# yamrom/smash-paper

Measured on AMD Instinct MI355X. Metric: reads/sec mapped+binned (hg19, 150 bp) at 1/2/4/8 MI355X; bit-exact bin counts, higher is better.
Workload: dtype u8/u64 (integer); 1 GPU; C3 hg19-shaped, 50 M x 150 bp SMASH reads per rank (25 M pairs, one run in batches), sample_bins/50000; genome=hg19, index_words=packed (SA / ISA hints, DESIGN section 3), genome_bp=3095693983, text_N=6191388016, pairs_per_rank=25000000, read_len=150, batch_pairs=12500000, bins=50000, parallelism=single GPU

## Files before the change

### smash-paper_amd/csrc/mam_sm.hpp

```cpp
#pragma once
#include "mam_device.hpp"

#ifndef PAD_KEEP
#define PAD_KEEP(x) asm volatile("" : "+v"(x))
#endif
#ifndef SM_KNOB
#define SM_KNOB(field, dflt) (dflt)
#endif
#ifndef SM_HOOK_BM
#define SM_HOOK_BM(mode, a1, a2)
#endif
#ifndef SM_HOOK_F
#define SM_HOOK_F(j, bits)
#endif
#ifndef SM_HOOK_BS
#define SM_HOOK_BS(size, depth)
#endif
#ifndef SM_HOOK_CMPBS
#define SM_HOOK_CMPBS(begin, sp, off)
#endif
#ifndef SM_HOOK_RUN
#define SM_HOOK_RUN(begin, kind, ext_l, ext_r)
#endif
#ifndef SM_HOOK_BYTE
#define SM_HOOK_BYTE(pos)
#endif
#ifndef SM_HOOK_PARK
#define SM_HOOK_PARK(a)
#endif
#ifndef SM_LOAD16
#define SM_LOAD16(a) ::smash::sm::load16u(a)
#endif
#ifndef SM_LOAD16ST
#define SM_LOAD16ST(a, st) SM_LOAD16(a)
#endif
#ifndef SM_LOADPF16
#define SM_LOADPF16(a) ::smash::sm::load16u(a)
#endif
#ifndef SM_LOADIDX
#define SM_LOADIDX(p, i) uint64_t((p)[i])
#endif
#ifndef SM_HOOK_PF
#define SM_HOOK_PF(a)
#endif
#ifndef SM_PERM
#define SM_PERM(s0, s1, sel) __builtin_amdgcn_perm(s0, s1, sel)
#endif

#ifndef SM_REGION
#define SM_REGION(k)                                                              \
  do {                                                                            \
    if (STATS) {                                                                  \
      const uint64_t am_ = __ballot(1);                                           \
      if (lane == uint32_t(__builtin_ctzll(am_))) atomicAdd(c.wave_stats + 64 + (k), 1ull); \
    }                                                                             \
  } while (0)
#endif

#ifndef SM_DMA_ROW
#define SM_DMA_ROW(dst, src, n, lane) ::smash::sm::dma_row(dst, src, n, lane)
#endif

namespace smash {
namespace sm {

#ifdef SM_DMA_ROW_HOST
__device__ __forceinline__ uint4 load16u(uint64_t a) {
  uint4 v;
  __builtin_memcpy(&v, reinterpret_cast<const uint8_t *>(a), 16);
  return v;
}
#else
typedef uint32_t sm_u32x4 __attribute__((ext_vector_type(4)));
typedef sm_u32x4 sm_u32x4_u __attribute__((aligned(1)));
typedef __attribute__((address_space(1))) const sm_u32x4_u glb_block16_t;
__device__ __forceinline__ uint4 load16u(uint64_t a) {
  const sm_u32x4 b = *reinterpret_cast<glb_block16_t *>(a);
  return make_uint4(b.x, b.y, b.z, b.w);
}
#endif

#ifndef SM_DMA_ROW_HOST
typedef __attribute__((address_space(3))) void lds_void_t;
typedef __attribute__((address_space(1))) const void glb_void_t;
__device__ __forceinline__ void dma_row(uint32_t *dst, const uint4 *src, uint32_t n, uint32_t lane) {
  if (lane < n)
    __builtin_amdgcn_global_load_lds((glb_void_t *)(src + lane), (lds_void_t *)dst, 16, 0, 0);
}
#endif

struct Geom {
  uint32_t w_raw;
  uint32_t w_row;
  uint32_t c_bad;
  uint32_t chunks;
};

__host__ __device__ constexpr uint32_t geo_row(uint32_t L) {
  return ((L + 11) / 4 + 3) / 4 * 4 < 8 ? 8u : ((L + 11) / 4 + 3) / 4 * 4;
}

inline Geom make_geom(uint32_t max_len) {
  Geom g;
  g.w_raw = (max_len + 11) / 4;
  g.w_row = (g.w_raw + 3) & ~3u;
  if (g.w_row < 8) g.w_row = 8;
  g.c_bad = max_len > 128 ? 2 : 1;
  g.chunks = g.c_bad + (g.w_row + 3) / 4;
  return g;
}


inline uint32_t prep_per_block(const Geom &g, uint64_t stride) {
  const uint64_t per = 24 * 1024 / (stride + 4 * (g.chunks * 4) + 8);
  return uint32_t(per < 1 ? 1 : per > 64 ? 64 : per);
}
__host__ __device__ inline uint32_t prep_in_words(uint64_t stride, uint32_t per) {
  return (uint32_t((per * stride + 8 + 3) / 4 + 10) + 3) & ~3u;
}
inline size_t prep_lds_bytes(const Geom &g, uint64_t stride, uint32_t per) {
  return size_t(prep_in_words(stride, per)) * 4 + size_t(per) * (g.chunks * 4) * 4;
}

__global__ __launch_bounds__(256) void k_prep(const uint8_t *__restrict__ seqs, uint64_t stride,
                                              const uint16_t *__restrict__ lens, uint32_t len0,
                                              uint64_t n, uint64_t it0, uint64_t it1, uint64_t it2,
                                              uint64_t it3, Geom g, uint32_t per,
                                              uint32_t *__restrict__ rec) {
  extern __shared__ uint32_t prep_lds[];
  const uint32_t rw = g.chunks * 4;
  const uint32_t G = 4 * g.c_bad;
  const uint64_t r0 = uint64_t(blockIdx.x) * per;
  if (r0 >= n) return;
  const uint32_t nr = uint32_t(n - r0 < per ? n - r0 : per);
  const uint64_t a0 = reinterpret_cast<uint64_t>(seqs + r0 * stride);
  const uint64_t a1 = reinterpret_cast<uint64_t>(seqs + (r0 + nr) * stride);
  const uint64_t w0 = a0 & ~uint64_t(3);
  const uint32_t nw = uint32_t(((a1 + 3) & ~uint64_t(3)) - w0) / 4;
  uint32_t *in = prep_lds;
  uint32_t *out = prep_lds + prep_in_words(stride, per);
  uint32_t k0 = 0;
  if ((w0 & 15) == 0) {
    const uint32_t n4 = nw / 4;
    for (uint32_t k = threadIdx.x; k < n4; k += blockDim.x)
      reinterpret_cast<uint4 *>(in)[k] = reinterpret_cast<const uint4 *>(w0)[k];
    k0 = 4 * n4;
  }
  for (uint32_t k = k0 + threadIdx.x; k < nw; k += blockDim.x)
    in[k] = reinterpret_cast<const uint32_t *>(w0)[k];
  for (uint32_t k = threadIdx.x; k < nr * rw / 4; k += blockDim.x)
    reinterpret_cast<uint4 *>(out)[k] = make_uint4(0, 0, 0, 0);
  __syncthreads();
  auto itx = [&](uint32_t b) {
    const uint64_t w = b < 64 ? it0 : b < 128 ? it1 : b < 192 ? it2 : it3;
    return uint32_t((w >> (b & 63)) & 1ull);
  };
  const uint32_t ia = itx('a'), ic = itx('c'), ig = itx('g'), iu = itx('t');
  for (uint32_t item = threadIdx.x; item < nr * G; item += blockDim.x) {
    const uint32_t t = item / G, gi = item - t * G;
    const uint32_t L = lens ? lens[r0 + t] : len0;
    if (32 * gi >= L) continue;
    const uint32_t boff = uint32_t(a0 - w0) + uint32_t(t * stride) + 32 * gi;
    const uint32_t wq = boff >> 2, sh = (boff & 3) * 8;
    uint32_t *o = out + t * rw;
    uint32_t bw = 0;
#pragma unroll
    for (uint32_t k = 0; k < 8; ++k) {
      uint32_t w = in[wq + k];
      if (sh) w = (w >> sh) | (in[wq + k + 1] << (32 - sh));
      const uint32_t i0 = 32 * gi + 4 * k;
#pragma unroll
      for (uint32_t j = 0; j < 4; ++j) {
        const uint32_t b = (w >> (8 * j)) & 0xFF;
        const bool live = i0 + j < L;
        if (!live) w &= ~(0xFFu << (8 * j));
        const uint32_t good = (b == 'a' ? ia : 0u) | (b == 'c' ? ic : 0u) |
                              (b == 'g' ? ig : 0u) | (b == 't' ? iu : 0u);
        bw |= uint32_t(live && !good) << (4 * k + j);
      }
      if (8 * gi + k < g.w_raw) o[4 * g.c_bad + 8 * gi + k] = w;
    }
    o[gi] = bw;
  }
  __syncthreads();
  uint4 *dst = reinterpret_cast<uint4 *>(rec + r0 * rw);
  for (uint32_t k = threadIdx.x; k < nr * rw / 4; k += blockDim.x)
    dst[k] = reinterpret_cast<const uint4 *>(out)[k];
}

__global__ __launch_bounds__(256) void k_prep_direct(const uint8_t *__restrict__ seqs,
                                                     uint64_t stride,
                                                     const uint16_t *__restrict__ lens,
                                                     uint32_t len0, uint32_t n, uint32_t ga,
                                                     uint64_t it0, uint64_t it1, uint64_t it2,
                                                     uint64_t it3, Geom g,
                                                     uint32_t *__restrict__ rec, uint32_t prio) {
#ifndef SM_DMA_ROW_HOST
  if (prio) __builtin_amdgcn_s_setprio(2);
#endif
  const uint32_t item = blockIdx.x * blockDim.x + threadIdx.x;
  if (item >= n * ga) return;
  const uint32_t r = item / ga;
  const uint32_t gi = item - r * ga;
  const uint32_t L = lens ? lens[r] : len0;
  uint32_t *o = rec + uint64_t(r) * (g.chunks * 4);
  uint32_t w8[8] = {0, 0, 0, 0, 0, 0, 0, 0};
  uint32_t bw = 0;
  if (32 * gi < L) {
    auto itx = [&](uint32_t b) {
      const uint64_t w = b < 64 ? it0 : b < 128 ? it1 : b < 192 ? it2 : it3;
      return uint32_t((w >> (b & 63)) & 1ull);
    };
    const uint32_t ia = itx('a'), ic = itx('c'), ig = itx('g'), iu = itx('t');
    const uint64_t end = reinterpret_cast<uint64_t>(seqs) + uint64_t(n) * stride;
    const uint64_t b0 = reinterpret_cast<uint64_t>(seqs) + uint64_t(r) * stride + 32 * gi;
    const uint64_t a16 = b0 & ~uint64_t(15);
    const uint32_t off = uint32_t(b0 & 15);
    uint32_t d[12];
#pragma unroll
    for (uint32_t k = 0; k < 3; ++k) {
      const uint4 v = a16 + 16 * k < end && (k < 2 || off) ? reinterpret_cast<const uint4 *>(a16)[k]
                                                          : make_uint4(0, 0, 0, 0);
      d[4 * k] = v.x; d[4 * k + 1] = v.y; d[4 * k + 2] = v.z; d[4 * k + 3] = v.w;
    }
    const uint32_t q = off >> 2, sh = (off & 3) * 8;
#pragma unroll
    for (uint32_t k = 0; k < 8; ++k) {
      const uint32_t lo = q == 0 ? d[k] : q == 1 ? d[k + 1] : q == 2 ? d[k + 2] : d[k + 3];
      const uint32_t hi = q == 0 ? d[k + 1] : q == 1 ? d[k + 2] : q == 2 ? d[k + 3] : d[k + 4];
      uint32_t w = sh ? (lo >> sh) | (hi << (32 - sh)) : lo;
      const uint32_t i0 = 32 * gi + 4 * k;
#pragma unroll
      for (uint32_t j = 0; j < 4; ++j) {
        const uint32_t b = (w >> (8 * j)) & 0xFF;
        const bool live = i0 + j < L;
        if (!live) w &= ~(0xFFu << (8 * j));
        const uint32_t good = (b == 'a' ? ia : 0u) | (b == 'c' ? ic : 0u) |
                              (b == 'g' ? ig : 0u) | (b == 't' ? iu : 0u);
        bw |= uint32_t(live && !good) << (4 * k + j);
      }
      w8[k] = 8 * gi + k < g.w_raw ? w : 0u;
    }
  }
  o[gi] = bw;
  uint32_t *raw = o + 4 * g.c_bad;
  if (8 * gi + 8 <= g.w_row) {
    reinterpret_cast<uint4 *>(raw + 8 * gi)[0] = make_uint4(w8[0], w8[1], w8[2], w8[3]);
    reinterpret_cast<uint4 *>(raw + 8 * gi)[1] = make_uint4(w8[4], w8[5], w8[6], w8[7]);
  } else {
#pragma unroll
    for (uint32_t k = 0; k < 8; ++k)
      if (8 * gi + k < g.w_row) raw[8 * gi + k] = w8[k];
  }
  if (gi == ga - 1) {
    for (uint32_t k = ga; k < 4 * g.c_bad; ++k) o[k] = 0;
    for (uint32_t k = 8 * ga; k < g.w_row; ++k) raw[k] = 0;
  }
}

inline uint32_t prep_groups(uint32_t max_len) { return (max_len + 31) / 32; }

enum : uint32_t { S_EXIT = 0, S_NEW, S_ALU, S_COPY, S_BM, S_KT, S_IDX, S_BYTE, S_CMP, S_USCAN,
                  S_EXL, S_EXR, S_EXB };
enum : uint32_t { O_SAPOS, O_SAPOS2, O_BS_SA, O_ISAJ, O_NS_SA2, O_NS_ISA2 };
enum : uint32_t { O_EXT = 0, O_BS };
enum : uint32_t { A_NONE = 0, A_BSP, A_BS, A_BS_DONE, A_XL_DONE, A_RUN_DONE, A_CHAIN_DONE,
                  A_EXPAND, A_AFTER, A_TOP, A_TRAV, A_DONE, A_EMIT, A_EXS,
                  A_TOPR };
enum : uint32_t { BS_INSERT = 0, BS_LEFT, BS_RIGHT };

__device__ __forceinline__ uint64_t lo64(const uint4 &v) { return uint64_t(v.x) | (uint64_t(v.y) << 32); }
__device__ __forceinline__ uint64_t hi64(const uint4 &v) { return uint64_t(v.z) | (uint64_t(v.w) << 32); }
__device__ __forceinline__ uint32_t dword_at(const uint4 &v, uint32_t i) {
  return i == 0 ? v.x : i == 1 ? v.y : i == 2 ? v.z : v.w;
}
__device__ __forceinline__ uint32_t byte_at(const uint4 &v, uint32_t o) {
  return (dword_at(v, o >> 2) >> (8 * (o & 3))) & 0xFF;
}
__device__ __forceinline__ uint64_t bytes8_at(const uint4 &v, uint32_t o) {
  const uint64_t lo = lo64(v), hi = hi64(v);
  if (o == 0) return lo;
  if (o < 8) return (lo >> (8 * o)) | (hi << (64 - 8 * o));
  if (o == 8) return hi;
  return hi >> (8 * (o - 8));
}
__device__ __forceinline__ uint32_t agree_block(const uint4 &v, uint32_t o, const uint8_t *P,
                                                uint32_t poff, uint32_t lim) {
  uint32_t k = agree8(bytes8_at(v, o), lds_load8(P, poff), lim < 8 ? lim : 8u);
  if (k == 8 && lim > 8) k += agree8(bytes8_at(v, o + 8), lds_load8(P, poff + 8), lim - 8);
  return k;
}
template <class F>
__device__ __forceinline__ uint32_t byte_mask(const uint4 &v, F f) {
  uint32_t m = 0;
#pragma unroll
  for (uint32_t i = 0; i < 16; ++i) {
    const uint32_t b = (dword_at(v, i >> 2) >> (8 * (i & 3))) & 0xFF;
    m |= uint32_t(f(b, i)) << i;
  }
  return m;
}

#ifndef SM_PK_SUB16
typedef unsigned short sm_u16x2 __attribute__((ext_vector_type(2)));
__device__ __forceinline__ uint32_t pk_sub16(uint32_t a, uint32_t b) {
  return __builtin_bit_cast(uint32_t, __builtin_bit_cast(sm_u16x2, a) - __builtin_bit_cast(sm_u16x2, b));
}
#define SM_PK_SUB16(a, b) ::smash::sm::pk_sub16(a, b)
#endif

__device__ __forceinline__ uint32_t gt4(uint32_t w, uint32_t te, uint32_t to) {
  const uint32_t e = SM_PERM(w, w, 0x0c020c00u), o = SM_PERM(w, w, 0x0c030c01u);
  const uint32_t r = SM_PERM(SM_PK_SUB16(to, o), SM_PK_SUB16(te, e), 0x0b090a08u);
  return ((r & 0x80808080u) * 0x00204081u) >> 28;
}
__device__ __forceinline__ uint32_t thr_mask(const uint4 &v, uint32_t base, bool desc) {
  const uint32_t bp = base * 0x00010001u, s4 = desc ? 0x00040004u : 0u;
  uint32_t te = bp - (desc ? 0x00020000u : 0u), to = bp - (desc ? 0x00030001u : 0u);
  uint32_t m = 0;
#pragma unroll
  for (uint32_t k = 0; k < 4; ++k) {
    m |= gt4(dword_at(v, k), te, to) << (4 * k);
    te -= s4;
    to -= s4;
  }
  return m;
}

struct FlagRef {
  uint32_t &f;
  uint32_t b;
  __device__ __forceinline__ operator bool() const { return (f >> b) & 1u; }
  __device__ __forceinline__ FlagRef &operator=(bool x) {
    f = (f & ~(1u << b)) | (uint32_t(x) << b);
    return *this;
  }
  __device__ __forceinline__ FlagRef &operator=(const FlagRef &o) { return *this = bool(o); }
};

struct Bad {
  uint32_t w0, w1, w2, w3, w4, w5, w6, w7;
  __device__ __forceinline__ uint32_t word(uint32_t i) const {
    uint32_t r = 0;
    r = i == 0 ? w0 : r; r = i == 1 ? w1 : r; r = i == 2 ? w2 : r; r = i == 3 ? w3 : r;
    r = i == 4 ? w4 : r; r = i == 5 ? w5 : r; r = i == 6 ? w6 : r; r = i == 7 ? w7 : r;
    return r;
  }
  __device__ __forceinline__ uint32_t bits(uint32_t a, uint32_t n) const {
    const uint32_t q = a >> 5, s = a & 31;
    const uint64_t x = (uint64_t(word(q + 1)) << 32) | word(q);
    const uint32_t y = uint32_t(x >> s);
    return n >= 32 ? y : (y & ((1u << n) - 1));
  }
  __device__ __forceinline__ uint64_t bits64(uint32_t a) const {
    const uint32_t q = a >> 5, s = a & 31;
    const uint64_t x = (uint64_t(word(q + 1)) << 32) | word(q);
    const uint64_t z = uint64_t(word(q + 2)) << 32;
    return (x >> s) | (s ? z << (32 - s) : 0ull);
  }
  __device__ __forceinline__ int32_t last(uint32_t a, uint32_t n) const {
    uint32_t e = a + n;
    while (e > a) {
      const uint32_t k = e - a < 32 ? e - a : 32u;
      const uint32_t s = e - k;
      const uint32_t y = bits(s, k);
      if (y) return int32_t(s + 31 - __builtin_clz(y));
      e = s;
    }
    return -1;
  }
};

__device__ __forceinline__ uint32_t byte4_codes(uint32_t w) {
  const uint32_t cb = SM_PERM(0x02000003u, 0x01000000u, w & 0x07070707u);
  return (cb * 0x40100401u) >> 24;
}

__device__ __forceinline__ uint64_t codes_raw(const uint32_t *R, uint32_t w_row, uint32_t p,
                                              uint32_t n) {
  const uint32_t q0 = p >> 2, qm = w_row - 6;
  const uint32_t q = q0 < qm ? q0 : qm, sh = p - 4 * q;
  uint32_t hi = byte4_codes(R[q]);
  hi = (hi << 8) | byte4_codes(R[q + 1]);
  hi = (hi << 8) | byte4_codes(R[q + 2]);
  hi = (hi << 8) | byte4_codes(R[q + 3]);
  const uint32_t lo = (byte4_codes(R[q + 4]) << 8) | byte4_codes(R[q + 5]);
  const uint64_t x = (uint64_t(hi) << 16) | lo;
  return (x >> (48 - 2 * (sh + n))) & ((1ull << (2 * n)) - 1);
}

__device__ __forceinline__ uint64_t codes_raw7(const uint32_t *R, uint32_t w_row, uint32_t p,
                                               uint32_t n) {
  const uint32_t q0 = p >> 2, qm = w_row - 7;
  const uint32_t q = q0 < qm ? q0 : qm, sh = p - 4 * q;
  uint32_t hi = byte4_codes(R[q]);
  hi = (hi << 8) | byte4_codes(R[q + 1]);
  hi = (hi << 8) | byte4_codes(R[q + 2]);
  uint32_t lo = byte4_codes(R[q + 3]);
  lo = (lo << 8) | byte4_codes(R[q + 4]);
  lo = (lo << 8) | byte4_codes(R[q + 5]);
  lo = (lo << 8) | byte4_codes(R[q + 6]);
  const uint64_t x = (uint64_t(hi) << 32) | lo;
  return (x >> (56 - 2 * (sh + n))) & ((1ull << (2 * n)) - 1);
}

template <class IdxT>
struct Ctx {
  const uint8_t *T;
  const IdxT *SA, *ISA;
  const uint8_t *L8, *U;
  const uint64_t *KT;
  uint64_t N;
  uint32_t logN, K, B, min_len;
  const uint4 *rec;
  uint32_t chunks, c_bad, w_row, w_raw;
  const uint4 *rows;
  uint32_t direct;
  uint32_t bad_tab_lo, bad_tab_hi;
  uint32_t lin_blocks;
  uint32_t pad;
  uint32_t mhint;
  uint32_t grab;
  uint32_t bm_dual;
  uint32_t pf;
  uint32_t u32;
  uint32_t f2;
  const uint16_t *lens;
  uint32_t len0, cap;
  uint64_t n_reads;
  uint64_t *out;
  uint32_t *n_out;
  unsigned long long *work;
  uint64_t lo, hi;
  unsigned long long *viol;
  uint64_t in_text[4];
  uint32_t *iters;
  unsigned long long *wave_stats;
};

template <class IdxT>
__device__ __forceinline__ uint64_t ia(const IdxT *a, uint64_t i) {
  return reinterpret_cast<uint64_t>(a + i);
}
template <class IdxT>
__device__ __forceinline__ uint64_t idx_val(const uint4 &v, uint32_t ao) {
  if (sizeof(IdxT) == 8) return (ao & 8) ? hi64(v) : lo64(v);
  return dword_at(v, ao >> 2);
}

__device__ __forceinline__ bool pk_below(uint64_t w, uint32_t b, uint32_t xd) {
  const uint32_t c = uint32_t(w >> b) & 127u;
  return c < xd && c < 127u;
}
__device__ __forceinline__ bool pk_above(uint64_t w, uint32_t b, uint32_t xd) {
  return (uint32_t(w >> b) & 127u) >= xd;
}
__device__ __forceinline__ uint32_t pk_char(uint32_t q) { return (0x74676361u >> (8 * q)) & 0xFFu; }
__device__ __forceinline__ uint64_t pk_map_hint(uint64_t w) {
  const uint32_t a = uint32_t(w >> 36) & 127u, b = uint32_t(w >> 43) & 127u;
  return (a < 127u && b < 127u) ? uint64_t((a > b ? a : b) + 1u) << 40 : 0ull;
}
__device__ __forceinline__ uint64_t pk_chain_hint(bool hit, uint32_t m) {
  return hit && m - 1u < 127u ? uint64_t(m) << kPkPosBits : 0ull;
}
__device__ __forceinline__ uint64_t pk_window(uint64_t w) {
  const uint32_t c = uint32_t(w >> 50);
  const uint32_t s0 = (c & 3u) | ((c << 6) & 0x300u) | ((c << 12) & 0x30000u) | ((c << 18) & 0x3000000u);
  const uint32_t s1 = ((c >> 8) & 3u) | ((c >> 2) & 0x300u) | ((c << 4) & 0x30000u) | 0x0c000000u;
  return uint64_t(SM_PERM(0u, 0x74676361u, s0)) | (uint64_t(SM_PERM(0u, 0x74676361u, s1)) << 32);
}

__device__ __forceinline__ uint32_t bad_nibble(uint32_t w, uint32_t tab_lo, uint32_t tab_hi,
                                               uint32_t live) {
  const uint32_t expect = SM_PERM(tab_hi, tab_lo, w & 0x07070707u);
  const uint32_t z = expect ^ w;
  const uint32_t nz = (((z & 0x7F7F7F7Fu) + 0x7F7F7F7Fu) | z) & 0x80808080u;
  const uint32_t nib = (nz * 0x00204081u) >> 28;
  return live >= 4 ? nib : nib & ((1u << live) - 1u);
}

__device__ inline Bad row_bad_mask(const uint32_t *row, uint32_t L, uint32_t tab_lo,
                                            uint32_t tab_hi) {
  uint32_t m[8] = {0, 0, 0, 0, 0, 0, 0, 0};
  for (uint32_t k = 0; 4 * k < L && k < 64; ++k)
    m[k >> 3] |= bad_nibble(row[k], tab_lo, tab_hi, L - 4 * k) << (4 * (k & 7));
  return Bad{m[0], m[1], m[2], m[3], m[4], m[5], m[6], m[7]};
}

inline void bad_table(const uint64_t in_text[4], uint32_t *lo, uint32_t *hi) {
  uint8_t t[8];
  for (uint32_t c = 0; c < 8; ++c) t[c] = uint8_t(0x80u | (c ^ 1u));
  const uint8_t letters[4] = {'a', 'c', 'g', 't'};
  for (uint8_t b : letters)
    if ((in_text[b >> 6] >> (b & 63)) & 1ull) t[b & 7] = b;
  *lo = uint32_t(t[0]) | uint32_t(t[1]) << 8 | uint32_t(t[2]) << 16 | uint32_t(t[3]) << 24;
  *hi = uint32_t(t[4]) | uint32_t(t[5]) << 8 | uint32_t(t[6]) << 16 | uint32_t(t[7]) << 24;
}

#ifndef SM_GEO_WPS
#define SM_GEO_WPS 1
#endif
template <class IdxT, int BLOCK, bool CHECK, bool STATS, bool PK = false, int GEO = 0>
__global__ __launch_bounds__(BLOCK, GEO ? SM_GEO_WPS : 1) void k_mam_sm(const Ctx<IdxT> c) {
  static_assert(GEO == 0 || (GEO >= 21 && GEO <= 255), "GEO is 0 or the read length");
  const uint32_t gK = GEO ? 16u : c.K, gMin = GEO ? 20u : c.min_len, gB = GEO ? 18u : c.B;
  const uint32_t gRow = GEO ? geo_row(GEO) : c.w_row, gLen0 = GEO ? uint32_t(GEO) : c.len0;
  const uint32_t gDirect = GEO ? 1u : c.direct, gPad = GEO ? 0u : c.pad, gMh = GEO ? 1u : c.mhint;
  const uint32_t gLogN = GEO ? 33u : c.logN, gCap = GEO ? uint32_t(GEO) - 19u : c.cap;
  const uint16_t *const gLens = GEO ? nullptr : c.lens;
  static_assert(!PK || sizeof(IdxT) == 8, "packed words are 8-byte elements");
  constexpr uint64_t PM = PK ? kPkPosMask : ~0ull;
  extern __shared__ uint32_t ldsw[];
  const uint64_t it0 = c.in_text[0], it1 = c.in_text[1], it2 = c.in_text[2], it3 = c.in_text[3];
  auto in_text = [&](uint32_t b) {
    const uint64_t w = b < 64 ? it0 : b < 128 ? it1 : b < 192 ? it2 : it3;
    return ((w >> (b & 63)) & 1ull) != 0;
  };
  const uint64_t N = c.N;
  uint32_t *row = ldsw + threadIdx.x * gRow;
  const uint8_t *P = reinterpret_cast<const uint8_t *>(row);
  const uint32_t lane = threadIdx.x & 63;
  const uint32_t row_live = 4 * lane < gLen0 ? (gLen0 - 4 * lane < 4 ? gLen0 - 4 * lane : 4u) : 0u;

  uint64_t q_next = 0, q_end = 0;
  uint32_t st = S_NEW, op = 0, pend = A_NONE;
  uint64_t addr = 0, addr2 = 0;
  uint32_t fl = 0;
  FlagRef need2{fl, 0};
  uint64_t rd = 0;
  uint32_t L = GEO ? uint32_t(GEO) : 0u, nem = 0;
  Bad bad{0, 0, 0, 0, 0, 0, 0, 0};
  uint32_t prefix = 0, depth = 0;
  uint64_t start = 0, end = 0, pos = 0;
  FlagRef have_pos{fl, 1};
  uint64_t lo = 0, hi = 0, bpos = 0, sp = 0, m = 0, bi = 0, es = 0, ee = 0;
  uint64_t &c0 = bpos, &c1 = sp;
  uint32_t lL = 0, lR = 0, best = 0, lc = 0, cbase = 0, cap = 0, bsm = 0, nblk = 0;
  FlagRef hit{fl, 2}, bm2{fl, 3}, skip_f{fl, 4}, xrun{fl, 5};
  FlagRef rdone{fl, 6};
  uint32_t fm = 0;
  uint32_t fk = 0, kp = 0, fj = 0, kx = 0xFFFFFFFFu;
  uint64_t klo = 1, khi = 0;
  FlagRef fdead{fl, 11};
  FlagRef ktr_set{fl, 7};
  FlagRef clean{fl, 8};
  FlagRef pf{fl, 9}, pfr{fl, 10};
  FlagRef xls{fl, 12}, xl1{fl, 13}, xrs{fl, 14}, xr1{fl, 15};
  FlagRef em{fl, 16};
  uint32_t dch = 0, j = 0, thresh = 0, xd = 0;
  uint32_t it = 0;
  uint64_t w_iters = 0, w_active = 0;
  auto uscan_start = [&](uint64_t p, uint32_t d) {
    dch = d; j = 1;
    addr = reinterpret_cast<uint64_t>(c.U + p + 1);
    addr2 = addr + 16;
    need2 = SM_KNOB(u32, 1u) && d - 1 > 16;
    st = S_USCAN;
  };
  auto bs_decide = [&](bool on, bool ranout, uint32_t pb, uint32_t tb) {
    bool left;
    if (bsm == BS_INSERT) {
      left = ranout || int8_t(pb) < int8_t(tb);
      const bool up = on && lc > best;
      best = up ? lc : best; bpos = up ? sp : bpos; bi = up ? m : bi;
    } else {
      left = (lc >= cap) == (bsm == BS_LEFT);
    }
    const bool l = on && left, r = on && !left;
    hi = l ? m : hi; lR = l ? lc : lR;
    lo = r ? m + 1 : lo; lL = r ? lc : lL;
  };
  auto bs_probe = [&]() -> bool {
    SM_HOOK_CMPBS(true, sp, cbase + lc);
    const uint32_t o = cbase + lc;
    bool dec = false;
    if (PK && ((sp >> kPkPosBits) & 7u) != 5u && o - gK < kPkWindow) {
      const uint32_t rem = cap - lc, nav = gK + kPkWindow - o;
      const uint32_t lim = rem < nav ? rem : nav;
      const uint64_t win = pk_window(sp) >> (8 * (o - gK));
      const uint32_t k = agree8(win, lds_load8(P, prefix + o), lim);
      lc += k;
      dec = k < lim || k == rem;
      if (dec) { SM_HOOK_CMPBS(false, sp, cbase + lc); }
      bs_decide(dec, k == rem, uint32_t(P[k == rem ? 0u : prefix + o + k]),
                uint32_t(win >> (8 * (k & 7))) & 0xFFu);
    }
    if (dec) {
      pf = false; pfr = false; need2 = false;
    } else {
      addr = reinterpret_cast<uint64_t>(c.T + (sp & PM) + cbase + lc);
      addr2 = ia(c.SA, (lo + m) >> 1);
      need2 = SM_KNOB(pf, 1u) && lo < m;
      pfr = SM_KNOB(pf, 1u) && m + 1 < hi;
      pf = SM_KNOB(pf, 1u) != 0;
      st = S_CMP; op = O_BS;
    }
    return dec;
  };
  auto lblock = [&](uint64_t e) { return reinterpret_cast<uint64_t>(c.L8 + (e >= 15 ? e - 15 : 0)); };
  auto ex_start = [&](uint64_t lb, uint64_t hb, bool ls, bool rs) {
    const bool l = !ls && es > lb, r = !rs && ee < hb;
    nblk = 0;
    rdone = !r;
    addr = l ? lblock(es) : reinterpret_cast<uint64_t>(c.L8 + ee + 1);
    addr2 = reinterpret_cast<uint64_t>(c.L8 + ee + 1);
    need2 = l && r;
    st = l && r ? S_EXB : l ? S_EXL : S_EXR;
    return l || r;
  };

  auto isa_hints = [&](uint64_t wl, uint64_t wr) {
    const uint32_t d = depth;
    xls = pk_below(wl, 40, d) || (pk_above(wl, 40, d) && pk_below(wl, 33, d));
    xl1 = !pk_below(wl, 40, d);
    xrs = pk_below(wr, 47, d) || (pk_above(wr, 47, d) && pk_below(wr, 54, d));
    xr1 = !pk_below(wr, 47, d);
  };

  for (;;) {
    const uint64_t newm = __ballot(st == S_NEW);
    const uint32_t need = uint32_t(__popcll(newm));
    const uint64_t avail = q_end - q_next;
    const uint64_t live = __ballot(st != S_EXIT);
    if (live == 0) break;
    if (STATS) { w_iters += 1; w_active += __popcll(live); }
    const uint32_t st_ld = S_COPY + gDirect;
    if (CHECK && st >= st_ld &&
        (addr < c.lo || addr >= c.hi || (need2 && (addr2 < c.lo || addr2 >= c.hi)))) {
      if (atomicAdd(c.viol, 1ull) == 0) {
        c.viol[1] = st; c.viol[2] = op; c.viol[3] = addr; c.viol[4] = need2 ? addr2 : 0;
        c.viol[5] = prefix; c.viol[6] = depth; c.viol[7] = start; c.viol[8] = end; c.viol[9] = rd;
      }
      st = S_EXIT;
      need2 = false; pfr = false;
    }
    const bool ld1 = st >= st_ld, ld2 = need2, ld3 = pfr;
    const uint64_t amask = st >= S_BYTE ? ~uint64_t(0) : ~uint64_t(15);
    const uint64_t a1 = addr & amask, a2 = addr2 & (pf ? ~uint64_t(15) : amask);
    const uint64_t i3 = (m + 1 + hi) >> 1;
    uint4 v, v2;
    uint64_t v3;
    unsigned long long base = 0;
    uint32_t take = 0;
    if (newm && avail < need) take = need > SM_KNOB(grab, 16u) ? need : SM_KNOB(grab, 16u);
#ifdef SM_HOST_LANE
    v = ld1 ? SM_LOAD16ST(a1, st) : make_uint4(0, 0, 0, 0);
    v2 = !ld2 ? make_uint4(0, 0, 0, 0) : pf ? SM_LOADPF16(a2) : SM_LOAD16ST(a2, st);
    v3 = ld3 ? SM_LOADIDX(c.SA, i3) : 0;
#else
    const uint64_t idle = reinterpret_cast<uint64_t>(c.T);
    v = SM_LOAD16ST(ld1 ? a1 : idle, st);
    v2 = SM_LOAD16(ld2 ? a2 : idle);
    v3 = SM_LOADIDX(c.SA, ld3 ? i3 : 0);
#endif
    if (take && lane == uint32_t(__builtin_ctzll(newm)))
      base = atomicAdd(c.work, (unsigned long long)take);
#ifndef SM_HOST_LANE
    __builtin_amdgcn_s_waitcnt(0x0F70);
    asm volatile("" ::: "memory");
    if (!ld1) v = make_uint4(0, 0, 0, 0);
    if (!ld2) v2 = make_uint4(0, 0, 0, 0);
    if (!ld3) v3 = 0;
#endif
    if (gDirect) {
      uint64_t cm = __ballot(st == S_COPY);
      if (cm) {
        SM_REGION(27);
#ifdef SM_HOST_LANE
        if (st == S_COPY) bad = row_bad_mask(row, L, c.bad_tab_lo, c.bad_tab_hi);
#else
        while (cm) {
          const uint32_t ln = uint32_t(__builtin_ctzll(cm));
          cm &= cm - 1;
          const uint32_t w = row_live ? ldsw[ln * gRow + lane] : 0u;
          const uint32_t nib = row_live ? bad_nibble(w, c.bad_tab_lo, c.bad_tab_hi, row_live) : 0u;
          if (__ballot(nib != 0)) {
            uint32_t x = nib << (4 * (lane & 7));
            x |= __shfl_xor(x, 1, 64);
            x |= __shfl_xor(x, 2, 64);
            x |= __shfl_xor(x, 4, 64);
            const uint32_t m0 = __shfl(x, 0, 64), m1 = __shfl(x, 8, 64), m2 = __shfl(x, 16, 64),
                           m3 = __shfl(x, 24, 64), m4 = __shfl(x, 32, 64), m5 = __shfl(x, 40, 64),
                           m6 = __shfl(x, 48, 64), m7 = __shfl(x, 56, 64);
            if (lane == ln) bad = Bad{m0, m1, m2, m3, m4, m5, m6, m7};
          }
        }
#endif
      }
    }
    bool fresh = false;
    if (newm) {
      if (take) base = __shfl(base, int(__builtin_ctzll(newm)), 64);
      if (st == S_NEW) {
        fresh = true;
        const uint32_t r = uint32_t(__popcll(newm & ((1ull << lane) - 1)));
        rd = r < avail ? q_next + r : base + (r - avail);
        if (rd >= c.n_reads) {
          st = S_EXIT;
        } else {
          L = gLens ? gLens[rd] : gLen0;
          addr = reinterpret_cast<uint64_t>(c.rec + rd * c.chunks);
          addr2 = addr + 16;
          need2 = !gDirect && c.c_bad > 1;
          pf = false; pfr = false;
          bad = Bad{0, 0, 0, 0, 0, 0, 0, 0};
          prefix = 0; depth = 0; start = 0; end = N - 1; have_pos = false; nem = 0;
          skip_f = false; fm = 0; ktr_set = false;
          fk = 0; kp = 0; kx = 0xFFFFFFFFu; fdead = false;
          st = S_COPY;
        }
      }
      if (take) { q_next = base + (need - avail); q_end = base + take; }
      else q_next += need;
      uint64_t fm_ = __ballot(fresh && st == S_COPY);
      if (fm_) SM_REGION(26);
      while (fm_) {
        const uint32_t ln = uint32_t(__builtin_ctzll(fm_));
        fm_ &= fm_ - 1;
        const uint64_t rl = __shfl(rd, int(ln), 64);
        if (gDirect)
          SM_DMA_ROW(ldsw + ln * gRow, c.rows + rl * (gRow >> 2), gRow >> 2, lane);
        else
          SM_DMA_ROW(ldsw + ln * gRow, c.rec + rl * c.chunks + c.c_bad, c.chunks - c.c_bad, lane);
      }
    }
    if (st < S_ALU || fresh) continue;
    if (STATS) {
      ++it;
      atomicAdd(c.wave_stats + 2 + (st == S_IDX ? 16 + op : st == S_CMP ? 40 + op : st), 1ull);
    }
#ifdef SM_TRACE
    if (st != S_COPY)
      printf("it %u st %u op %u prefix %u depth %u [%llu,%llu] pos %llu hp %d\n", it, st, op, prefix,
             depth, (unsigned long long)start, (unsigned long long)end, (unsigned long long)pos,
             int(have_pos));
#endif
    const uint32_t ao = st >= S_BYTE ? 0u : uint32_t(addr) & 15;
    uint32_t a = A_NONE;
    SM_REGION(0);
    uint32_t mv = 0, mv2 = 0;
    if (st >= S_USCAN) {
      const bool us = st == S_USCAN;
      const uint32_t base = us ? dch - j - 1 : xd - 1;
      mv = thr_mask(v, base, us);
      mv2 = thr_mask(v2, us ? base - 16 : base, us);
    }

    const uint32_t st0 = st;
    if (st0 == S_ALU) {
      SM_REGION(1);
      a = pend;
    }
    if (st0 == S_COPY) {
      SM_REGION(2);
      if (!gDirect) {
        bad.w0 = v.x; bad.w1 = v.y; bad.w2 = v.z; bad.w3 = v.w;
        bad.w4 = v2.x; bad.w5 = v2.y; bad.w6 = v2.z; bad.w7 = v2.w;
      }
      need2 = false;
      clean = (bad.w0 | bad.w1 | bad.w2 | bad.w3 | bad.w4 | bad.w5 | bad.w6 | bad.w7) == 0;
      a = A_TOP;
    }
    if (st0 == S_BM) {
      SM_REGION(3);
      const bool two = need2;
      need2 = false;
      if (SM_KNOB(bm_dual, 3u) == 3) {
        const uint32_t nb = 2 * (gK + 4);
        auto entry_bits = [&](const uint4 &e, uint64_t cc) {
          const uint64_t f48 = kt_filter(lo64(e), hi64(e));
          const uint32_t l1 = uint32_t(cc >> (nb - 2)) & 3, l0 = uint32_t(cc >> (nb - 4)) & 3;
          const uint32_t r1 = uint32_t(cc >> 2) & 3, r2 = uint32_t(cc) & 3;
          return (uint32_t(f48 >> (32 + 4 * l1 + l0)) & 1u) |
                 ((uint32_t(f48 >> (16 + 4 * l0 + r1)) & 1u) << 1) |
                 ((uint32_t(f48 >> (4 * r1 + r2)) & 1u) << 2);
        };
        const uint32_t bits = entry_bits(v, c0);
        SM_HOOK_F(fj, bits);
        fk |= (7u << fj) | (bits << (16 + fj));
        fdead = bits != 7u;
        if (two) {
          const uint32_t bits2 = entry_bits(v2, c1);
          SM_HOOK_F(fj + 3, bits2);
          fk |= (7u << (fj + 3)) | (bits2 << (19 + fj));
          fdead = fdead || bits2 != 7u;
        }
        kx = kp + fj + 2;
        klo = lo64(v) & kKtMask;
        khi = hi64(v) & kKtMask;
        a = A_TOP;
      } else {
        const uint64_t cc = bm2 ? c0 : c1;
        const bool pa = (lo64(v) >> (40 + (cc & 15))) & 1ull;
        const bool pb = !SM_KNOB(bm_dual, 3u) || ((lo64(v2) >> (40 + (c0 & 15))) & 1ull);
        if (SM_KNOB(bm_dual, 3u) == 2) {
          const uint32_t D = gMin - gB;
          const uint32_t fm0 = fm;
          SM_HOOK_BM(fm, pa, pb);
          uint32_t adv = 0, nfm = 0;
          bool pass = false;
          if (fm == 0) {
            if (!pa) { adv = D + 1; nfm = 1; }
            else if (!pb) adv = 1;
            else pass = true;
          } else if (fm == 1) {
            if (!pa && !pb) { adv = 2 * D + 2; nfm = 1; }
            else if (!pa) { adv = D + 1; nfm = 2; }
            else nfm = 2;
          } else {
            if (!pb) adv = 2;
            else if (!pa) adv = 1;
            else pass = true;
          }
          if (pass) {
            skip_f = true; fm = 1;
            m = (fm0 == 0 ? c0 : c1) >> (2 * (gB - gK));
            ktr_set = true;
          } else {
            fm = nfm;
            if (adv) { depth = 0; start = 0; end = N - 1; have_pos = false; prefix += adv; }
          }
          a = A_TOP;
        } else if (!pa && !bm2) {
          depth = 0; start = 0; end = N - 1; have_pos = false;
          prefix += gMin - gB + 1;
          a = A_TOP;
        } else if (!pa || !pb) {
          depth = 0; start = 0; end = N - 1; have_pos = false; ++prefix; a = A_TOP;
        } else if (!bm2 && !SM_KNOB(bm_dual, 3u)) {
          bm2 = true;
          addr = reinterpret_cast<uint64_t>(c.KT + 2 * (c0 >> 4));
        } else {
          skip_f = true;
          a = A_TOP;
        }
      }
    }
    if (st0 == S_KT) {
      SM_REGION(4);
      const uint64_t l0 = lo64(v) & kKtMask, h0 = hi64(v) & kKtMask;
      if (l0 <= h0) { depth = gK; start = l0; end = h0; have_pos = false; }
      a = A_TRAV;
    }
    if (st0 == S_IDX) {
      SM_REGION(5);
      const uint64_t iv = idx_val<IdxT>(v, ao);
      const uint64_t iv2 = idx_val<IdxT>(v2, uint32_t(addr2) & 15);
      if (PK && (op == O_ISAJ || op == O_NS_ISA2)) isa_hints(iv, op == O_ISAJ ? iv : iv2);
      const uint32_t op0 = op;
      const bool sap = op0 <= O_SAPOS2, bsa = op0 == O_BS_SA, isj = op0 == O_ISAJ;
      const bool ns1 = op0 == O_NS_SA2, ns2 = op0 == O_NS_ISA2, se = isj || ns2;
      const uint64_t p1 = iv & PM, p2 = iv2 & PM;
      pos = sap ? iv : pos;
      sp = bsa ? iv : sp;
      start = se ? p1 : start;
      end = isj ? p1 : ns2 ? p2 : end;
      fl = sap ? fl | 2u : se ? fl & ~(2u | uint32_t(ns2)) : fl;
      addr = ns1 ? ia(c.ISA, p1 + 1) : addr;
      addr2 = ns1 ? ia(c.ISA, p2 + 1) : addr2;
      op = ns1 ? uint32_t(O_NS_ISA2) : op0;
      prefix += uint32_t(ns2);
      constexpr uint32_t nxt = A_TRAV | (A_AFTER << 4) | (A_BSP << 8) | (A_EXPAND << 12) |
                               (A_NONE << 16) | (A_EXPAND << 20);
      a = (nxt >> (4 * op0)) & 15u;
      a = ns2 && depth == 0 ? uint32_t(A_TOPR) : a;
    }
    if (st0 == S_BYTE) {
      SM_REGION(6);
      SM_HOOK_BYTE(pos & PM);
      em = P[prefix - 1] != uint8_t(byte_at(v, ao));
      a = A_EMIT;
    }
    if (st0 == S_CMP) {
      SM_REGION(7);
      const bool tn2 = need2 && !pf;
      const uint32_t off = prefix + (op == O_BS ? cbase : depth) + lc;
      const uint32_t rem = op == O_BS ? cap - lc : L - off;
      const uint32_t lim = rem < 16 ? rem : 16u;
      uint32_t k = agree_block(v, 0, P, off, lim);
      if (tn2 && k == lim && k < rem) {
        const uint32_t lim2 = rem - k < 16 ? rem - k : 16u;
        k += agree_block(v2, 0, P, off + k, lim2);
      }
      const uint32_t got = tn2 ? (rem < 32 ? rem : 32u) : lim;
      const bool had_pf = pf;
      pf = false; pfr = false;
      lc += k;
      if (k == got && k < rem) {
        addr += k;
        addr2 = addr + 16;
        need2 = rem - k > 16;
      } else if (op == O_EXT) {
        need2 = false;
        depth += lc; lc = 0;
        a = A_AFTER;
      } else {
        SM_HOOK_CMPBS(false, sp, cbase + lc);
        need2 = false;
        const uint32_t tbyte = k < 16 ? byte_at(v, k) : byte_at(v2, k - 16);
        bs_decide(true, k == rem, k == rem ? 0u : uint32_t(P[off + k]), tbyte);
        const bool left = hi == m;
        if (had_pf && lo < hi) {
          m = (lo + hi) >> 1;
          SM_HOOK_PF(ia(c.SA, m));
          sp = left ? idx_val<IdxT>(v2, uint32_t(m * sizeof(IdxT)) & 15) : v3;
          lc = lL < lR ? lL : lR;
          a = A_BSP;
        } else {
          a = A_BS;
        }
      }
    }
    if (st0 == S_USCAN) {
      SM_REGION(8);
      bool fin = false;
#pragma unroll
      for (uint32_t h = 0; h < 2; ++h) {
        if (fin || (h == 1 && !need2)) break;
        const uint32_t D = dch - j;
        const uint32_t lim = D < 16 ? D : 16u;
        const uint32_t inr = (1u << lim) - 1;
        const uint32_t hm = (h ? mv2 : mv) & inr;
        if (hm) {
          j += uint32_t(__builtin_ctz(hm)); hit = true; fin = true;
        } else {
          j += lim;
          if (j >= dch) { hit = false; fin = true; }
        }
      }
      if (fin) {
        need2 = false;
        a = A_CHAIN_DONE;
      } else {
        addr += need2 ? 32 : 16;
        addr2 = addr + 16;
        need2 = SM_KNOB(u32, 1u) && dch - j > 16;
      }
    }
    if (st0 >= S_EXL) {
      SM_REGION(9);
      const uint64_t lb = xrun ? start : 0, hb = xrun ? end : N - 1;
      auto side = [&](uint32_t mask, uint32_t o, bool left, bool &more) {
        const uint64_t room = left ? es - lb : hb - ee;
        const uint32_t w = left ? o + 1 : 16 - o;
        const uint32_t lim = room < uint64_t(w) ? uint32_t(room) : w;
        const uint32_t below = ~mask & 0xFFFFu;
        const uint32_t win = left ? (((1u << lim) - 1) << (o + 1 - lim)) : (((1u << lim) - 1) << o);
        const uint32_t sm = below & win;
        const uint32_t k = sm ? (left ? o - (31 - __builtin_clz(sm)) : uint32_t(__builtin_ctz(sm)) - o)
                              : lim;
        more = !sm && uint64_t(k) < room;
        return k;
      };
      bool moreL = false, moreR = false;
      if (st != S_EXR)
        es -= side(mv, uint32_t(es - (addr - reinterpret_cast<uint64_t>(c.L8))), true, moreL);
      if (st != S_EXL) {
        const bool b2 = st == S_EXB;
        ee += side(b2 ? mv2 : mv, 0u, false, moreR);
        if (b2) rdone = !moreR;
      }
      need2 = false;
      const bool left = st != S_EXR;
      const bool more = left ? moreL : moreR;
      if (!more) {
        a = left ? A_XL_DONE : A_RUN_DONE;
      } else if (++nblk < SM_KNOB(lin_blocks, 8u)) {
        addr = left ? lblock(es) : reinterpret_cast<uint64_t>(c.L8 + ee + 1);
        st = left ? S_EXL : S_EXR;
      } else {
        bsm = left ? BS_LEFT : BS_RIGHT;
        if (left) { lo = lb; hi = es; lL = 0; lR = cap; }
        else { lo = ee + 1; hi = hb + 1; lL = cap; lR = 0; }
        a = A_BS;
      }
    }

    if (gPad) {
      uint32_t x = uint32_t(addr);
      for (uint32_t k = 0; k < gPad; ++k) {
        x += k;
        PAD_KEEP(x);
      }
    }

    if (a == A_BSP) {
      SM_REGION(28);
      a = bs_probe() ? A_BS : A_NONE;
    }
    if (a == A_BS) {
      SM_REGION(10);
      if (lo < hi) {
        m = (lo + hi) >> 1;
        lc = lL < lR ? lL : lR;
        addr = ia(c.SA, m);
        st = S_IDX; op = O_BS_SA;
        a = A_NONE;
      } else {
        a = A_BS_DONE;
      }
    }
    if (a == A_BS_DONE) {
      SM_REGION(11);
      lc = 0;
      const bool bl = bsm == BS_LEFT, br = bsm == BS_RIGHT, run = bsm == BS_INSERT && best != 0;
      es = bl ? lo : run ? bi : es;
      ee = br ? lo - 1 : run ? bi : ee;
      a = bl ? uint32_t(A_XL_DONE) : br ? uint32_t(A_RUN_DONE) : uint32_t(A_AFTER);
      if (run) {
        xd = depth + best; xrun = true;
        cbase = depth; cap = best;
        SM_HOOK_RUN(true, 1, 0, 0);
        xls = PK && pk_below(bpos, 36, xd); xrs = PK && pk_below(bpos, 43, xd);
        a = A_EXS;
      }
    }
    if (a == A_EXPAND) {
      SM_REGION(15);
      thresh = 2u * depth * gLogN;
      xd = depth; xrun = false;
      cbase = 0; cap = depth;
      es = start; ee = end;
      SM_HOOK_RUN(true, 0, 0, 0);
      if (PK) {
        if (xls && xl1) es = start - 1;
        if (xrs && xr1) ee = end + 1;
      }
      a = A_EXS;
    }
    if (a == A_EXS) {
      SM_REGION(29);
      a = ex_start(xrun ? start : 0, xrun ? end : N - 1, xls, xrs) ? A_NONE : A_RUN_DONE;
    }
    if (a == A_XL_DONE) {
      SM_REGION(12);
      const uint64_t hb = xrun ? end : N - 1;
      nblk = 0;
      if (!xrun && start - es >= thresh) {
        SM_HOOK_RUN(false, 0, start - es, 99);
        a = A_TOPR;
      } else if (ee < hb && !rdone) {
        addr = reinterpret_cast<uint64_t>(c.L8 + ee + 1);
        st = S_EXR;
        a = A_NONE;
      } else {
        a = A_RUN_DONE;
      }
    }
    if (a == A_RUN_DONE) {
      SM_REGION(13);
      SM_HOOK_RUN(false, xrun ? 1 : 0, xrun ? bi - es : start - es, xrun ? ee - bi : ee - end);
      if (xrun) {
        start = es; end = ee; depth = xd; pos = bpos; have_pos = start == end;
        a = A_AFTER;
      } else {
        a = (start - es) + (ee - end) >= thresh ? A_TOPR : A_TOP;
        start = es; end = ee;
      }
    }
    if (a == A_CHAIN_DONE) {
      SM_REGION(14);
      if (em) {
        if (nem < gCap)
          c.out[rd * gCap + nem] =
              pack_match(pos & PM, prefix, dch) |
              (PK && gMh ? pk_map_hint(pos) | pk_chain_hint(hit, dch - j + 1) : 0ull);
        ++nem;
      }
      prefix += j;
      if (!hit) {
        a = A_TOPR;
      } else {
        depth = dch - j;
        addr = ia(c.ISA, (pos & PM) + j);
        st = S_IDX; op = O_ISAJ;
        a = A_NONE;
      }
    }
    if (a == A_TOP || a == A_TOPR) {
      SM_REGION(17);
      if (a != A_TOP) {
        SM_REGION(31);
        depth = 0; start = 0; end = N - 1; have_pos = false;
        a = A_TOP;
      }
      uint32_t kpos = ~0u;
      const uint32_t bp0 = prefix;
      uint64_t bwin = 0;
      if (!clean) bwin = bad.bits64(prefix);
      auto badw = [&](uint32_t p, uint32_t n) {
        return uint32_t(bwin >> (p - bp0)) & ((1u << n) - 1u);
      };
      bool proceed = skip_f || depth >= gMin;
      const bool ktr = skip_f && ktr_set;
      skip_f = false; ktr_set = false;
      if (prefix >= L || (!proceed && prefix + gMin > L)) {
        a = A_DONE;
      } else if (!proceed) {
        SM_REGION(24);
        int32_t kb = -1;
        const uint32_t B = gB;
        const uint32_t D = gMin - B;
        if (!clean) {
          SM_REGION(20);
          kb = bad.last(prefix, gMin);
          while (kb >= 0 && in_text(P[kb]))
            kb = bad.last(prefix, uint32_t(kb) - prefix);
        }
        if (kb >= 0) {
          depth = 0; start = 0; end = N - 1; have_pos = false;
          prefix = uint32_t(kb) + 1;
          fm = 0;
        } else if (SM_KNOB(bm_dual, 3u) == 3) {
          if (B != gK + 2 || B > gMin || D + 3 > 16) {
            proceed = true;
          } else {
            const uint32_t sh = prefix - kp;
            uint32_t kn = sh < 16 ? (fk & 0xFFFFu) >> sh : 0u;
            uint32_t pr = sh < 16 ? (fk >> 16) >> sh : 0u;
            kp = prefix;
            const uint32_t A = kn & ~pr;
            uint32_t kill = A;
            for (uint32_t i = 1; i <= D; ++i) kill |= A >> i;
            const uint32_t adv = uint32_t(__builtin_ctz(~kill));
            if (adv) {
              prefix += adv; kp = prefix;
              kn >>= adv; pr >>= adv;
              depth = 0; start = 0; end = N - 1; have_pos = false;
            }
            fk = kn | (pr << 16);
            const uint32_t need = (2u << D) - 1;
            if (prefix + gMin > L) {
              a = A_DONE;
            } else if ((kn & pr & need) == need) {
              proceed = true;
            } else {
              const uint32_t W = gK + 4;
              const uint32_t u = uint32_t(__builtin_ctz(~kn & need));
              auto ok_at = [&](uint32_t jj) {
                return prefix + jj + W <= L && badw(prefix + jj, W) == 0;
              };
              uint32_t jq = (fdead && ((kn & need) >> u) == 0) ? D : u;
              if (!ok_at(jq)) jq = u;
              if (!ok_at(jq) && u >= 1) jq = u - 1;
              if (!ok_at(jq) && u >= 2) jq = u - 2;
              if (!ok_at(jq)) {
                proceed = true;
              } else {
                SM_REGION(21);
                fj = jq;
                kpos = prefix + jq;
                need2 = SM_KNOB(f2, 2u) && (SM_KNOB(f2, 2u) == 1 || fdead) && jq + 6 <= 16 &&
                        ((kn >> (jq + 3)) & 7u) != 7u && ok_at(jq + 3);
                st = S_BM;
                a = A_NONE;
              }
            }
          }
        } else {
          const uint32_t sM = prefix + 2 * D + 1;
          bool okP = true, okQ = true;
          bool okP1 = prefix + 1 + B <= L, okM = sM + B <= L;
          if (!clean) {
            okP = bad.bits(prefix, B) == 0;
            okQ = bad.bits(prefix + D, B) == 0;
            okP1 = okP1 && bad.bits(prefix + 1, B) == 0;
            okM = okM && bad.bits(sM, B) == 0;
          }
          uint32_t s1 = prefix + D, s2 = prefix;
          bool ok = okQ && okP;
          if (SM_KNOB(bm_dual, 3u) == 2 && fm == 1 && okQ && okM) {
            s2 = sM; ok = true;
          } else if (SM_KNOB(bm_dual, 3u) == 2 && fm == 2 && okP && okP1) {
            s1 = prefix; s2 = prefix + 1; ok = true;
          } else {
            fm = 0;
          }
          if (B > 0 && B <= gMin && ok) {
            const uint32_t lo_s = s1 < s2 ? s1 : s2, hi_s = s1 < s2 ? s2 : s1;
            const uint32_t span = hi_s + B - lo_s;
            if (span <= 21) {
              SM_REGION(21);
              const uint64_t X = codes_raw(row, gRow, lo_s, span);
              const uint64_t mk = (1ull << (2 * B)) - 1;
              c1 = (X >> (2 * (lo_s + span - s1 - B))) & mk;
              c0 = (X >> (2 * (lo_s + span - s2 - B))) & mk;
            } else {
              SM_REGION(22);
              c0 = codes_raw(row, gRow, s2, B);
              c1 = codes_raw(row, gRow, s1, B);
            }
            addr = reinterpret_cast<uint64_t>(c.KT + 2 * (c1 >> 4));
            st = S_BM; bm2 = false;
            if (SM_KNOB(bm_dual, 3u)) { addr2 = reinterpret_cast<uint64_t>(c.KT + 2 * (c0 >> 4)); need2 = true; }
            a = A_NONE;
          } else {
            proceed = true;
            fm = 1;
          }
        }
      }
      if (a == A_TOP && proceed) {
        if (depth == 0 && prefix + gK <= L && badw(prefix, gK) == 0) {
          if (kx == prefix) {
            SM_REGION(25);
            if (klo <= khi) { depth = gK; start = klo; end = khi; have_pos = false; }
            a = A_TRAV;
          } else {
            SM_REGION(23);
            if (ktr) addr = reinterpret_cast<uint64_t>(c.KT + 2 * m);
            else kpos = prefix;
            st = S_KT;
            a = A_NONE;
          }
        } else {
          a = A_TRAV;
        }
      }
      if (kpos != ~0u) {
        const uint64_t kmask = (1ull << (2 * gK)) - 1;
        const uint64_t cw = codes_raw7(row, gRow, kpos, gK + 7);
        const bool fb = st == S_BM;
        if (fb) {
          c0 = cw >> 6;
          c1 = cw & ((1ull << (2 * (gK + 4))) - 1);
          addr2 = reinterpret_cast<uint64_t>(c.KT + 2 * ((c1 >> 4) & kmask));
        }
        addr = reinterpret_cast<uint64_t>(c.KT + 2 * ((cw >> (fb ? 10 : 14)) & kmask));
      }
    }
    if (a == A_TRAV) {
      SM_REGION(18);
      if (depth >= L || prefix + depth >= L) {
        a = A_AFTER;
      } else {
        a = A_NONE;
        lo = start; hi = end + 1; lL = 0; lR = 0; best = 0;
        bsm = BS_INSERT; cbase = depth; cap = L - prefix - depth;
        m = (lo + hi) >> 1;
        lc = 0;
        if (start == end) {
          if (!have_pos) {
            addr = ia(c.SA, start);
            st = S_IDX; op = O_SAPOS;
          } else {
            addr = reinterpret_cast<uint64_t>(c.T + (pos & PM) + depth);
            addr2 = addr + 16;
            need2 = L - prefix - depth > 16;
            st = S_CMP; op = O_EXT;
          }
        } else {
          SM_HOOK_BS(end - start + 1, depth);
          addr = ia(c.SA, m);
          st = S_IDX; op = O_BS_SA;
        }
      }
    }
    if (a == A_AFTER) {
      SM_REGION(16);
      if (depth <= 1) {
        ++prefix;
        a = A_TOPR;
      } else {
        a = A_NONE;
        if (start != end) {
          --depth;
          addr = ia(c.SA, start); addr2 = ia(c.SA, end); need2 = true;
          st = S_IDX; op = O_NS_SA2;
        } else if (!have_pos) {
          addr = ia(c.SA, start);
          st = S_IDX; op = O_SAPOS2;
        } else if (depth >= gMin && prefix != 0 && (pos & PM) != 0 &&
                   (!PK || ((pos >> kPkPosBits) & 7u) >= 4u)) {
          addr = reinterpret_cast<uint64_t>(c.T + (pos & PM) - 1);
          st = S_BYTE;
        } else {
          em = depth >= gMin &&
               (!PK || prefix == 0 || (pos & PM) == 0 ||
                P[prefix - 1] != pk_char(uint32_t(pos >> kPkPosBits) & 3u));
          a = A_EMIT;
        }
      }
    }
    if (a == A_EMIT) {
      SM_REGION(30);
      uscan_start(pos & PM, depth);
      a = A_NONE;
    }
    if (a == A_DONE) {
      SM_REGION(19);
      c.n_out[rd] = nem;
      if (STATS && c.iters) c.iters[rd] = it;
      it = 0;
      st = S_NEW;
    } else if (a != A_NONE) {
      SM_HOOK_PARK(a);
      pend = a;
      st = S_ALU;
    }
  }
  if (STATS && lane == 0) {
    atomicAdd(c.wave_stats, (unsigned long long)w_iters);
    atomicAdd(c.wave_stats + 1, (unsigned long long)w_active);
  }
}

}
}
```

Before: 516.0 million reads/s.

## Prefetch work-queue batches ahead and hand new reads over at iteration end

Read assignment moves out of the main loop body into an end-of-iteration hand_over step. A second reserve queue is refilled through the atomic work counter whenever the local queue falls below a low-water mark, so the atomic's latency overlaps the next iteration instead of stalling lanes that need a read. Lanes that pick up a read now go on to ALU work in the same iteration rather than idling one round. Broadcasts use readlane/readfirstlane instead of shfl. The cost is extra queue state and a 'dry' flag that must handle exit correctly.

```diff
diff --git a/smash-paper_amd/csrc/mam_sm.hpp b/smash-paper_amd/csrc/mam_sm.hpp
--- a/smash-paper_amd/csrc/mam_sm.hpp
+++ b/smash-paper_amd/csrc/mam_sm.hpp
@@ -88,6 +88,24 @@
     __builtin_amdgcn_global_load_lds((glb_void_t *)(src + lane), (lds_void_t *)dst, 16, 0, 0);
 }
 #endif
+
+__device__ __forceinline__ uint64_t lane0_u64(uint64_t v) {
+#ifdef SM_DMA_ROW_HOST
+  return v;
+#else
+  return uint64_t(uint32_t(__builtin_amdgcn_readfirstlane(int(uint32_t(v))))) |
+         uint64_t(uint32_t(__builtin_amdgcn_readfirstlane(int(uint32_t(v >> 32))))) << 32;
+#endif
+}
+__device__ __forceinline__ uint64_t lane_u64(uint64_t v, uint32_t ln) {
+#ifdef SM_DMA_ROW_HOST
+  (void)ln;
+  return v;
+#else
+  return uint64_t(uint32_t(__builtin_amdgcn_readlane(int(uint32_t(v)), int(ln)))) |
+         uint64_t(uint32_t(__builtin_amdgcn_readlane(int(uint32_t(v >> 32)), int(ln)))) << 32;
+#endif
+}
 
 struct Geom {
   uint32_t w_raw;
@@ -500,6 +518,7 @@
 #ifndef SM_GEO_WPS
 #define SM_GEO_WPS 1
 #endif
+constexpr uint32_t kLowWater = 4;
 template <class IdxT, int BLOCK, bool CHECK, bool STATS, bool PK = false, int GEO = 0>
 __global__ __launch_bounds__(BLOCK, GEO ? SM_GEO_WPS : 1) void k_mam_sm(const Ctx<IdxT> c) {
   static_assert(GEO == 0 || (GEO >= 21 && GEO <= 255), "GEO is 0 or the read length");
@@ -522,7 +541,9 @@
   const uint32_t lane = threadIdx.x & 63;
   const uint32_t row_live = 4 * lane < gLen0 ? (gLen0 - 4 * lane < 4 ? gLen0 - 4 * lane : 4u) : 0u;
 
-  uint64_t q_next = 0, q_end = 0;
+  uint64_t q_next = 0, r_next = 0;
+  uint32_t q_n = 0, r_n = 0;
+  bool dry = false;
   uint32_t st = S_NEW, op = 0, pend = A_NONE;
   uint64_t addr = 0, addr2 = 0;
   uint32_t fl = 0;
@@ -617,10 +638,57 @@
     xr1 = !pk_below(wr, 47, d);
   };
 
-  for (;;) {
+  auto hand_over = [&]() {
+    const uint64_t newm = __ballot(st == S_NEW);
+    if (!newm) return;
+    const uint32_t need = uint32_t(__popcll(newm));
+    const uint32_t avail = q_n + r_n;
+    const uint32_t r = uint32_t(__popcll(newm & ((1ull << lane) - 1)));
+    bool got = false;
+    if (st == S_NEW) {
+      if (r < avail) {
+        rd = r < q_n ? q_next + r : r_next + (r - q_n);
+        if (rd >= c.n_reads) {
+          st = S_EXIT;
+        } else {
+          got = true;
+          L = gLens ? gLens[rd] : gLen0;
+          addr = reinterpret_cast<uint64_t>(c.rec + rd * c.chunks);
+          addr2 = addr + 16;
+          need2 = !gDirect && c.c_bad > 1;
+          pf = false; pfr = false;
+          bad = Bad{0, 0, 0, 0, 0, 0, 0, 0};
+          prefix = 0; depth = 0; start = 0; end = N - 1; have_pos = false; nem = 0;
+          skip_f = false; fm = 0; ktr_set = false;
+          fk = 0; kp = 0; kx = 0xFFFFFFFFu; fdead = false;
+          st = S_COPY;
+        }
+      } else if (dry) {
+        st = S_EXIT;
+      }
+    }
+    const uint32_t used = need < avail ? need : avail;
+    if (used < q_n) {
+      q_next += used; q_n -= used;
+    } else {
+      q_next = r_next + (used - q_n); q_n = avail - used; r_n = 0;
+    }
+    uint64_t fm_ = __ballot(got);
+    if (fm_) SM_REGION(26);
+    while (fm_) {
+      const uint32_t ln = uint32_t(__builtin_ctzll(fm_));
+      fm_ &= fm_ - 1;
+      const uint64_t rl = lane_u64(rd, ln);
+      if (gDirect)
+        SM_DMA_ROW(ldsw + ln * gRow, c.rows + rl * (gRow >> 2), gRow >> 2, lane);
+      else
+        SM_DMA_ROW(ldsw + ln * gRow, c.rec + rl * c.chunks + c.c_bad, c.chunks - c.c_bad, lane);
+    }
+  };
+
+  for (;; hand_over()) {
     const uint64_t newm = __ballot(st == S_NEW);
     const uint32_t need = uint32_t(__popcll(newm));
-    const uint64_t avail = q_end - q_next;
     const uint64_t live = __ballot(st != S_EXIT);
     if (live == 0) break;
     if (STATS) { w_iters += 1; w_active += __popcll(live); }
@@ -642,7 +710,8 @@
     uint64_t v3;
     unsigned long long base = 0;
     uint32_t take = 0;
-    if (newm && avail < need) take = need > SM_KNOB(grab, 16u) ? need : SM_KNOB(grab, 16u);
+    if (!dry && r_n == 0 && q_n < need + kLowWater)
+      take = need > SM_KNOB(grab, 16u) ? need : SM_KNOB(grab, 16u);
 #ifdef SM_HOST_LANE
     v = ld1 ? SM_LOAD16ST(a1, st) : make_uint4(0, 0, 0, 0);
     v2 = !ld2 ? make_uint4(0, 0, 0, 0) : pf ? SM_LOADPF16(a2) : SM_LOAD16ST(a2, st);
@@ -653,8 +722,7 @@
     v2 = SM_LOAD16(ld2 ? a2 : idle);
     v3 = SM_LOADIDX(c.SA, ld3 ? i3 : 0);
 #endif
-    if (take && lane == uint32_t(__builtin_ctzll(newm)))
-      base = atomicAdd(c.work, (unsigned long long)take);
+    if (take && lane == 0) base = atomicAdd(c.work, (unsigned long long)take);
 #ifndef SM_HOST_LANE
     __builtin_amdgcn_s_waitcnt(0x0F70);
     asm volatile("" ::: "memory");
@@ -688,43 +756,12 @@
 #endif
       }
     }
-    bool fresh = false;
-    if (newm) {
-      if (take) base = __shfl(base, int(__builtin_ctzll(newm)), 64);
-      if (st == S_NEW) {
-        fresh = true;
-        const uint32_t r = uint32_t(__popcll(newm & ((1ull << lane) - 1)));
-        rd = r < avail ? q_next + r : base + (r - avail);
-        if (rd >= c.n_reads) {
-          st = S_EXIT;
-        } else {
-          L = gLens ? gLens[rd] : gLen0;
-          addr = reinterpret_cast<uint64_t>(c.rec + rd * c.chunks);
-          addr2 = addr + 16;
-          need2 = !gDirect && c.c_bad > 1;
-          pf = false; pfr = false;
-          bad = Bad{0, 0, 0, 0, 0, 0, 0, 0};
-          prefix = 0; depth = 0; start = 0; end = N - 1; have_pos = false; nem = 0;
-          skip_f = false; fm = 0; ktr_set = false;
-          fk = 0; kp = 0; kx = 0xFFFFFFFFu; fdead = false;
-          st = S_COPY;
-        }
-      }
-      if (take) { q_next = base + (need - avail); q_end = base + take; }
-      else q_next += need;
-      uint64_t fm_ = __ballot(fresh && st == S_COPY);
-      if (fm_) SM_REGION(26);
-      while (fm_) {
-        const uint32_t ln = uint32_t(__builtin_ctzll(fm_));
-        fm_ &= fm_ - 1;
-        const uint64_t rl = __shfl(rd, int(ln), 64);
-        if (gDirect)
-          SM_DMA_ROW(ldsw + ln * gRow, c.rows + rl * (gRow >> 2), gRow >> 2, lane);
-        else
-          SM_DMA_ROW(ldsw + ln * gRow, c.rec + rl * c.chunks + c.c_bad, c.chunks - c.c_bad, lane);
-      }
-    }
-    if (st < S_ALU || fresh) continue;
+    if (take) {
+      r_next = lane0_u64(base);
+      r_n = take;
+      dry = r_next + take >= c.n_reads;
+    }
+    if (st < S_ALU) continue;
     if (STATS) {
       ++it;
       atomicAdd(c.wave_stats + 2 + (st == S_IDX ? 16 + op : st == S_CMP ? 40 + op : st), 1ull);
```

Result: no change. 519.9 million reads/s, median of 6 (+0.8%).
